# darioShar/DLPM

Measured on AMD Instinct MI355X. Metric: samples/sec at T=1000 (CIFAR-10 32x32, alpha=1.7), higher is better.
Workload: dtype f32 (1x1 / stride-2 convolutions: fp32 operands split exactly into 3 bf16 planes, bf16 MFMA products, fp32 accumulate)

## Files before the change

### dlpm_amd/csrc/conv_wino4.hip

```cpp
#include <cstdlib>
#include <type_traits>

#include "conv.h"
#include "gn_stats.h"

namespace dlpm {
namespace {

typedef float floatx4 __attribute__((ext_vector_type(4)));

constexpr int F4_TILES = 16;
constexpr int F4_NQ = 128;
constexpr int F4_KC = 8;
constexpr int F4_RAWPIX = 576;
constexpr int F4_PRLD = F4_KC + 4;
constexpr int F4_NT = 512;
constexpr int F4_QNIT = (F4_RAWPIX * 2 + F4_NT - 1) / F4_NT;
constexpr int F4_RAWBUF = F4_RAWPIX * F4_PRLD + 16;
constexpr int F4_RAWPIX_N = 400;
constexpr int F4_RAWBUF_N = F4_RAWPIX_N * F4_PRLD + 16;
constexpr int f4_nq_of(int cout) { return cout % 128 == 0 ? 128 : cout % 64 == 0 ? 64 : 32; }
constexpr int F4_CFS = 16 * 2 * F4_KC;
constexpr int F4_VBUF = 36 * F4_TILES * F4_KC;
#ifndef F4_RING_DEPTH
// ... 106 lines not shown
#pragma unroll
        for (int c = 0; c < 6; c++) Tb[c] = f4_bt_outer<5>(d, c);
        f4_v_row_out(Tb, vb + 5 * 3 * vpp, vpp);
    }
}

__device__ __forceinline__ void f4_at(float m0, float m1, float m2, float m3, float m4, float m5, float &y0, float &y1, float &y2, float &y3) {
    const float s12 = m1 + m2, d12 = m1 - m2, s34 = m3 + m4, d34 = m3 - m4;
    y0 = m0 + s12 + s34;
    y1 = fmaf(PB, d34, PA * d12);
    y2 = fmaf(PB2, s34, PA2 * s12);
    y3 = fmaf(PB3, d34, PA3 * d12) + m5;
}
__device__ __forceinline__ void f4_out_tile(const floatx4 (&acc)[36], int r, float (&Yt)[16]) {
    float Z[4][6];
#pragma unroll
    for (int b = 0; b < 6; b++)
        f4_at(acc[0 * 6 + b][r], acc[1 * 6 + b][r], acc[2 * 6 + b][r], acc[3 * 6 + b][r], acc[4 * 6 + b][r], acc[5 * 6 + b][r], Z[0][b], Z[1][b],
              Z[2][b], Z[3][b]);
#pragma unroll
    for (int i = 0; i < 4; i++) f4_at(Z[i][0], Z[i][1], Z[i][2], Z[i][3], Z[i][4], Z[i][5], Yt[i * 4 + 0], Yt[i * 4 + 1], Yt[i * 4 + 2], Yt[i * 4 + 3]);
}

template <int N>
__device__ __forceinline__ void f4_stats_lane(float K, float s1, float s2, float &mean, float &M2) {
    mean = K + s1 * (1.f / N);
    M2 = fmaxf(s2 - s1 * s1 * (1.f / N), 0.f);
}
template <int N>
__device__ __forceinline__ void f4_stats_merge(float K, float s1, float s2, int lane, float &mean, float &M2) {
    f4_stats_lane<N>(K, s1, s2, mean, M2);
    float na = (float)N;
#pragma unroll
    for (int sft = 16; sft <= 32; sft <<= 1) {
        const float om = __shfl_xor(mean, sft), oM2 = __shfl_xor(M2, sft);
        const float lo_m = (lane & sft) ? om : mean, hi_m = (lane & sft) ? mean : om;
        const float lo_M = (lane & sft) ? oM2 : M2, hi_M = (lane & sft) ? M2 : oM2;
        const float dd = hi_m - lo_m;
        mean = lo_m + dd * 0.5f;
        M2 = lo_M + hi_M + dd * dd * (na * 0.5f);
        na *= 2.f;
    }
}

__device__ __forceinline__ void f4_mfma4(float4 aa, float4 b, floatx4 &acc0, floatx4 &acc1) {
    acc0 = __builtin_amdgcn_mfma_f32_16x16x4f32(aa.x, b.x, acc0, 0, 0, 0);
    acc1 = __builtin_amdgcn_mfma_f32_16x16x4f32(aa.z, b.z, acc1, 0, 0, 0);
    acc0 = __builtin_amdgcn_mfma_f32_16x16x4f32(aa.y, b.y, acc0, 0, 0, 0);
    acc1 = __builtin_amdgcn_mfma_f32_16x16x4f32(aa.w, b.w, acc1, 0, 0, 0);
}
__device__ __forceinline__ void f4_mfma_pair(int pp, const float *asrc, int vpp, const float4 *wp, int lane, float4 (&aq)[2], float4 (&bq)[F4_RING],
                                             floatx4 (&acc)[36]) {
    constexpr int AHEAD = F4_RING - 1;
    if (pp == 0) aq[0] = *reinterpret_cast<const float4 *>(asrc);
    if (pp + AHEAD < 18) bq[(pp + AHEAD) % F4_RING] = wp[(pp + AHEAD) * 64 + lane];
    if (pp + 1 < 18) aq[(pp + 1) & 1] = *reinterpret_cast<const float4 *>(asrc + (pp + 1) * vpp);
    f4_mfma4(aq[pp & 1], bq[pp % F4_RING], acc[2 * pp], acc[2 * pp + 1]);
}

__device__ __forceinline__ float4 f4_affine4(float4 x, float4 ca, float4 cb) {
    return make_float4(fmaf(x.x, ca.x, cb.x), fmaf(x.y, ca.y, cb.y), fmaf(x.z, ca.z, cb.z), fmaf(x.w, ca.w, cb.w));
}
__device__ __forceinline__ float4 f4_silu4(float4 x) { return make_float4(silu_f(x.x), silu_f(x.y), silu_f(x.z), silu_f(x.w)); }
__device__ __forceinline__ float4 f4_affine_silu4(float4 x, float4 ca, float4 cb) { return f4_silu4(f4_affine4(x, ca, cb)); }
template <int W, int PRLD>
__device__ __forceinline__ int f4_item_pack(int pix, int ch) {
    constexpr int RW = W + 2;
    const int ry = pix / RW, rx = pix - ry * RW;
    const int iy = ry - 1, ix = rx - 1;
    const bool pad = iy < 0 || iy >= W || ix < 0 || ix >= W;
    const int lo = pix * PRLD + ch + 4 * (ry >> 2);
    return pix >= RW * RW ? (1 << 25) : (lo | (pad ? (1 << 24) : ((iy * W + ix) << 14)));
}
__device__ __forceinline__ int f4_item_lds(int iv) { return iv & 16383; }
__device__ __forceinline__ int f4_item_src(int iv) { return (iv >> 14) & 1023; }
__device__ __forceinline__ bool f4_item_pad(int iv) { return iv & (1 << 24); }
__device__ __forceinline__ bool f4_item_none(int iv) { return iv & (1 << 25); }

__device__ __forceinline__ void fs_v_row_out(const float2 (&T)[5], int ra, float *vb, int vpp) {
    const float2 e1 = f4_bt_part<1>(T[2], T[4]), o1 = f4_bt_part<1>(T[1], T[3]);
    const float2 e2 = f4_bt_part<3>(T[2], T[4]), o2 = f4_bt_part<3>(T[1], T[3]);
// ... 3 lines not shown
        const int pos = 5 * ra + rb;
        *reinterpret_cast<float2 *>(vb + (pos >> 1) * vpp + (pos & 1) * 2) = v[rb];
    }
}
template <class D>
__device__ __forceinline__ void fs_transform_rp(int rp, const D &d, float *vb, int vpp) {
    float2 Ta[5], Tb[5];
    if (rp == 0) {
#pragma unroll
        for (int c = 0; c < 5; c++) Ta[c] = f4_bt_outer<0>(d, c);
        fs_v_row_out(Ta, 0, vb, vpp);
    } else if (rp == 1) {
#pragma unroll
        for (int c = 0; c < 5; c++) f4_bt_mid<1>(d, c, Ta[c], Tb[c]);
        fs_v_row_out(Ta, 1, vb, vpp);
        fs_v_row_out(Tb, 2, vb, vpp);
    } else {
#pragma unroll
        for (int c = 0; c < 5; c++) f4_bt_mid<3>(d, c, Ta[c], Tb[c]);
        fs_v_row_out(Ta, 3, vb, vpp);
        fs_v_row_out(Tb, 4, vb, vpp);
    }
}
__device__ __forceinline__ void fs_out_tile(const floatx4 (&acc)[25], int r, float (&Yt)[16]) {
    float Z[4][5];
#pragma unroll
    for (int b = 0; b < 5; b++)
        f4_at(acc[0 * 5 + b][r], acc[1 * 5 + b][r], acc[2 * 5 + b][r], acc[3 * 5 + b][r], acc[4 * 5 + b][r], 0.f, Z[0][b], Z[1][b], Z[2][b], Z[3][b]);
#pragma unroll
    for (int i = 0; i < 4; i++) f4_at(Z[i][0], Z[i][1], Z[i][2], Z[i][3], Z[i][4], 0.f, Yt[i * 4 + 0], Yt[i * 4 + 1], Yt[i * 4 + 2], Yt[i * 4 + 3]);
}

template <bool UPS, int QN = F4_QNIT, int NW = 8>
__global__ void __launch_bounds__((NW + (NW == 8 ? 0 : NW == 4 ? 3 : 2)) * 64, NW == 2 ? 2 : 1) k_conv3x3_wino4(ConvLaunch p_in, int bh_in, int bw_in, int nimg_in) {
    constexpr bool HELP = NW != 8;
    constexpr int NH = NW == 8 ? 0 : NW == 4 ? 3 : 2;
    constexpr int F4_NT = (NW + NH) * 64, F4_NQ = NW * 16;
    constexpr int F4_RAWBUF = NW == 8 ? dlpm::F4_RAWBUF : F4_RAWBUF_N;
    ConvLaunch p = p_in;
    const int bh = bh_in, bw = bw_in, nimg = nimg_in;
    extern __shared__ __attribute__((aligned(16))) float wsm[];
    float *V = wsm;
    float *raw = wsm + 2 * F4_VBUF;
    float *Cf = raw + 2 * F4_RAWBUF;

    DLPM_PHASE_DECL;
#ifdef DLPM_PHASE_TIMING
    const long long _c0 = clock64(), _r0 = wall_clock64();
#endif
#ifdef DLPM_PHASE_TIMING
    long long _wait = 0;
#endif
    const int tid = threadIdx.x, lane = tid & 63, wave = tid >> 6;
    const bool mfma_wave = !HELP || wave < NW;
    const int li = lane & 15, lk = lane >> 4;
    const int W = p.Wout, H = p.Hout, TW = W >> 2, TH = H >> 2;
    const int Ws = UPS ? (W >> 1) : W, Hs = UPS ? (H >> 1) : H;
    const int Cin = p.C0 + p.C1;
    int nch = Cin / F4_KC, kb = 0;
    unsigned bid = blockIdx.x, nblk = gridDim.x;
    if constexpr (HELP) {
        if (p.ksplit > 1) {
            nblk = gridDim.x / p.ksplit;
            const int ks = (int)(blockIdx.x / nblk);
            bid = blockIdx.x - (unsigned)ks * nblk;
            nch /= p.ksplit;
            kb = ks * nch;
            p.out += (int64_t)ks * p.B * H * W * p.Cout;
        }
    }
    const int ntn = p.Cout / F4_NQ;
    const int nmb = nblk / ntn;
    const int mb = bid % nmb, n0 = (bid / nmb) * F4_NQ;
    int img0, ty0, tx0, blk_in_img = 0;
    if (nimg == 1) {
        const int bpr = TW / bw, bpi = (TH / bh) * bpr;
        img0 = mb / bpi;
        blk_in_img = mb - img0 * bpi;
        ty0 = (blk_in_img / bpr) * bh;
        tx0 = (blk_in_img % bpr) * bw;
    } else {
        img0 = mb * nimg;
        ty0 = tx0 = 0;
    }
    const int RH = UPS ? 2 * bh + 2 : 4 * bh + 2, RW = UPS ? 2 * bw + 2 : 4 * bw + 2;
    const int oy = UPS ? 2 * ty0 - 1 : 4 * ty0 - 1, ox = UPS ? 2 * tx0 - 1 : 4 * tx0 - 1;
    const int rpi = RH * RW, npix = nimg * rpi;

    const int squad = tid & 1;
    auto pix_of = [&](int it) { return it == 1 ? (F4_NT / 2) + ((F4_NT - 1 - tid) >> 1) : it * (F4_NT / 2) + (tid >> 1); };
    const bool skewed = !UPS && nimg == 1 && bh <= 4;
    int off[QN], lo[QN];
#pragma unroll
    for (int it = 0; it < QN; it++) {
        const int pix = pix_of(it);
        const int img = min(pix / rpi, nimg - 1), r = pix - img * rpi;
        const int ry = r / RW, rx = r - ry * RW;
        const int iy = oy + ry, ix = ox + rx;
        const bool pad = iy < 0 || iy >= Hs || ix < 0 || ix >= Ws || (img0 + img) >= p.B;
        off[it] = pix >= npix ? -2 : (pad ? -1 : (((img0 + img) * Hs + iy) * Ws + ix));
        lo[it] = (pix * F4_PRLD + squad * 4 + (skewed ? 4 * (ry >> 2) : 0)) | ((img * 2 * F4_KC + squad * 4) << 16);
    }
    const bool has_coef = p.coefA != nullptr;
    const int cf_img = tid >> 2, cf_isb = (tid >> 1) & 1;
    const bool cf_mine = has_coef && tid < nimg * 4;
    const float *cf_base = has_coef ? ((cf_isb ? p.coefB : p.coefA) + (int64_t)min(img0 + cf_img, p.B - 1) * Cin + kb * F4_KC + squad * 4) : nullptr;
    float4 xr[QN], cfr = make_float4(0.f, 0.f, 0.f, 0.f);
    auto load_raw_into = [&](float4 (&dst)[QN], int chunk) {
        const int c = (kb + chunk) * F4_KC + squad * 4;
        const bool first = c < p.C0;
        const float *sb = first ? p.src0 + c : p.src1 + (c - p.C0);
        const int ld = first ? p.C0 : p.C1;
#pragma unroll
        for (int it = 0; it < QN; it++) dst[it] = *reinterpret_cast<const float4 *>(sb + (int64_t)max(off[it], 0) * ld);
    };
    auto load_coef = [&](int chunk) {
        if (cf_mine) cfr = *reinterpret_cast<const float4 *>(cf_base + chunk * F4_KC);
    };
    auto store_coef = [&](int slot) {
        if (cf_mine) *reinterpret_cast<float4 *>(Cf + slot * F4_CFS + cf_img * 2 * F4_KC + cf_isb * F4_KC + squad * 4) = cfr;
    };
    auto store_raw_item = [&](int slot, int it) {
        if (off[it] == -2) return;
        float *rb = raw + slot * F4_RAWBUF;
        float4 x = xr[it];
        if (has_coef) {
            const float4 ca = *reinterpret_cast<const float4 *>(Cf + slot * F4_CFS + (lo[it] >> 16));
            const float4 cb = *reinterpret_cast<const float4 *>(Cf + slot * F4_CFS + (lo[it] >> 16) + F4_KC);
            x = f4_affine4(x, ca, cb);
        }
        if (p.act_silu) x = f4_silu4(x);
        if (off[it] < 0) x = make_float4(0.f, 0.f, 0.f, 0.f);
        *reinterpret_cast<float4 *>(rb + (lo[it] & 0xffff)) = x;
    };
    auto store_raw = [&](int slot) {
#pragma unroll
        for (int it = 0; it < QN; it++) store_raw_item(slot, it);
    };

    int rbase, vofs;
    {
        const int tile = lane & 15, pair = lane >> 4;
        const int timg = tile / (bh * bw), r = tile - timg * (bh * bw);
        const int ty = r / bw, tx = r - ty * bw;
        rbase = (timg * rpi + (UPS ? 2 : 4) * ty * RW + (UPS ? 2 : 4) * tx) * F4_PRLD + pair * 2 + (skewed ? 4 * ty : 0);
        vofs = (pair * F4_TILES + tile) * 4;
    }
    auto transform_rp = [&](int slot, int rp) {
        f4_transform_rp(rp, F4Patch<UPS, F4_PRLD>{raw + slot * F4_RAWBUF + rbase, RW, skewed}, V + slot * F4_VBUF + vofs, 4 * F4_TILES * 4);
    };
    auto transform = [&](int slot) {
        if (HELP) {
            if (mfma_wave) return;
            if (NH == 3) {
                transform_rp(slot, wave - NW);
            } else if (wave == NW) {
                transform_rp(slot, 0);
                transform_rp(slot, 1);
            } else {
                transform_rp(slot, 2);
            }
        } else if (wave < 3) {
            transform_rp(slot, wave);
        }
    };

    const float4 *__restrict__ wp = reinterpret_cast<const float4 *>(p.w_wino4) +
// ... 61 lines not shown
            if (pp + F4_AAHEAD < 18)
                aq[(pp + F4_AAHEAD) % (F4_AAHEAD + 1)] = *reinterpret_cast<const float4 *>(ab + (pp + F4_AAHEAD) * (4 * F4_TILES * 4));
            if (F4_PRIO) __builtin_amdgcn_s_setprio(0);
            f4_mfma4(aq[pp % (F4_AAHEAD + 1)], bq[pp % F4_RING], acc[2 * pp], acc[2 * pp + 1]);
            if (F4_PRIO) __builtin_amdgcn_s_setprio(1);
        }
        }
        store_coef(nxt);
#ifdef DLPM_PHASE_TIMING
        const long long _w0 = clock64();
#endif
        __syncthreads();
#ifdef DLPM_PHASE_TIMING
        _wait += clock64() - _w0;
#endif
    }
    if (F4_PRIO) __builtin_amdgcn_s_setprio(0);
    DLPM_PHASE(p, 9);
    if (HELP && !mfma_wave) return;
#if defined(DLPM_PHASE_TIMING) && !defined(DLPM_PHASE_DEFER)
    if (p.phase && lane == 0) atomicAdd(p.phase + 16 + wave, (unsigned long long)_wait);
#endif

    const int64_t pix0 = ((int64_t)img0 * H + 4 * ty0) * W + 4 * tx0;
    const int ch = n0 + 16 * wave + li;
    const float bias_v = p.bias ? p.bias[ch] : 0.f;
    const bool has_res = p.res0 != nullptr;
    const bool res_first = __builtin_amdgcn_readfirstlane(n0 + 16 * wave) < p.R0;
    const float *res_u = has_res ? (res_first ? p.res0 : p.res1 - p.R0) : nullptr;
    const int res_ld = res_first ? p.R0 : p.Cout - p.R0;
    const int lbw = 31 - __builtin_clz(bw), lbhw = 31 - __builtin_clz(bh * bw);
    float *__restrict__ out_blk = p.out + pix0 * p.Cout;
    const float *__restrict__ res_blk = has_res ? res_u + pix0 * res_ld : nullptr;
    const bool img_stats = p.stats_out != nullptr && nimg == 4 && bh * bw == 4;
    const bool do_stats = (p.stats_out != nullptr && nimg == 1) || img_stats;
    float K = 0.f, s1 = 0.f, s2 = 0.f;
    float rs_all[HELP ? 4 : 1][16] = {};
#pragma unroll
    for (int r = 0; r < 4; r++) {
        const int tile = 4 * lk + r;
        const int timg = tile >> lbhw, ty = (tile & (bh * bw - 1)) >> lbw, tx = tile & (bw - 1);
        const int tpix = (timg * H + 4 * ty) * W + 4 * tx;
        const bool ok = img0 + timg < p.B;
        float rs[16];
        const uint32_t bo_o = (uint32_t)(tpix * p.Cout + ch) * 4u, bo_r = (uint32_t)(tpix * res_ld + ch) * 4u;
        if (HELP) {
            if (r == 0 && has_res) {
#pragma unroll
                for (int rr = 0; rr < 4; rr++) {
                    const int t2 = 4 * lk + rr;
                    const int tp2 = ((t2 >> lbhw) * H + 4 * ((t2 & (bh * bw - 1)) >> lbw)) * W + 4 * (t2 & (bw - 1));
                    const uint32_t b2 = (uint32_t)(tp2 * res_ld + ch) * 4u;
                    const bool ok2 = img0 + (t2 >> lbhw) < p.B;
#pragma unroll
                    for (int k = 0; k < 16; k++)
                        rs_all[rr][k] = ok2 ? *reinterpret_cast<const float *>(reinterpret_cast<const char *>(res_blk + ((k >> 2) * W + (k & 3)) * res_ld) + b2) : 0.f;
                }
            }
#pragma unroll
            for (int k = 0; k < 16; k++) rs[k] = rs_all[r][k];
        } else if (has_res && ok) {
#pragma unroll
            for (int i = 0; i < 4; i++)
#pragma unroll
                for (int j = 0; j < 4; j++)
                    rs[i * 4 + j] = *reinterpret_cast<const float *>(reinterpret_cast<const char *>(res_blk + (i * W + j) * res_ld) + bo_r);
        }
        float Yt[16];
        f4_out_tile(acc, r, Yt);
        if (!ok) continue;
#pragma unroll
        for (int i = 0; i < 4; i++) {
            const float *y = Yt + 4 * i;
#pragma unroll
            for (int j = 0; j < 4; j++) {
                float v = y[j] + bias_v;
                if (has_res) v += rs[i * 4 + j];
                if (do_stats) {
                    if (r == 0 && i == 0 && j == 0) K = v;
                    const float dd = v - K;
                    s1 += dd;
                    s2 = fmaf(dd, dd, s2);
                }
                *reinterpret_cast<float *>(reinterpret_cast<char *>(out_blk + (i * W + j) * p.Cout) + bo_o) = v;
            }
        }
    }
    if (img_stats) {
        if (img0 + lk < p.B) {
            float mean, M2;
            f4_stats_lane<64>(K, s1, s2, mean, M2);
            p.stats_out[(int64_t)(img0 + lk) * p.Cout + ch] = make_float2(mean, M2);
        }
    } else if (do_stats) {
        float mean, M2;
        f4_stats_merge<64>(K, s1, s2, lane, mean, M2);
        if (lk == 0) p.stats_out[((int64_t)img0 * ((H * W) / 256) + blk_in_img) * p.Cout + ch] = make_float2(mean, M2);
    }
    DLPM_PHASE(p, 10);
    DLPM_PHASE_FLUSH(p, 8);
#ifdef DLPM_PHASE_DEFER
    if (p.phase && lane == 0) atomicAdd(p.phase + 16 + wave, (unsigned long long)_wait);
#endif
#ifdef DLPM_PHASE_TIMING
    if (p.phase && tid == 0) {
        atomicAdd(p.phase + 11, 1ull);
        atomicAdd(p.phase + 12, (unsigned long long)(clock64() - _c0));
        atomicAdd(p.phase + 13, (unsigned long long)(wall_clock64() - _r0));
    }
#endif
}

constexpr int FS_PP = 12;
constexpr int FS_FRAGS = 13;
constexpr int FS_VPP = 4 * F4_TILES * 4;
constexpr int FS_VBUF = FS_FRAGS * FS_VPP;
constexpr int FS_RAWPIX = 352;
constexpr int FS_RAWBUF = FS_RAWPIX * F4_PRLD + 16;
constexpr int FS_PAD = 16;
constexpr int FS_S0 = 4, FS_X = 9;
static_assert(FS_PP % F4_RING == 0, "a fragment's ring slot must not depend on the phase");

__global__ void __launch_bounds__(F4_NT, 1) k_conv3x3_wino4sp(ConvLaunch p_in, int bh_in, int bw_in, int nimg_in) {
    constexpr int QN = 2;
    ConvLaunch p = p_in;
    const int bh = bh_in, bw = bw_in, nimg = nimg_in;
    extern __shared__ __attribute__((aligned(16))) float wsm[];
    float *V = wsm;
    float *raw = wsm + 2 * FS_VBUF;
    float *Cf = raw + 2 * FS_RAWBUF;

    DLPM_PHASE_DECL;
#ifdef DLPM_PHASE_TIMING
    const long long _c0 = clock64(), _r0 = wall_clock64();
#endif
    const int tid = threadIdx.x, lane = tid & 63, wave = tid >> 6;
    const int li = lane & 15, lk = lane >> 4;
    const int W = p.Wout, H = p.Hout, Ws = p.Win, Hs = p.Hin, TW = Ws >> 2, TH = Hs >> 2;
    const int Cin = p.C0 + p.C1;
    const int nch = Cin / F4_KC;
    const unsigned bid = blockIdx.x;
    const int ntn = p.Cout / F4_NQ;
    const int nmb = (gridDim.x >> 2) / ntn;
    const int cls = bid & 3, mb = (bid >> 2) % nmb, nt = (bid >> 2) / nmb;
    const int ca = cls >> 1, cb = cls & 1, n0 = nt * F4_NQ;
    int img0, ty0, tx0, blk_in_img = 0;
    const int bpr = TW / bw, bpi = (TH / bh) * bpr;
    if (nimg == 1) {
        img0 = mb / bpi;
        blk_in_img = mb - img0 * bpi;
        ty0 = (blk_in_img / bpr) * bh;
        tx0 = (blk_in_img % bpr) * bw;
    } else {
        img0 = mb * nimg;
        ty0 = tx0 = 0;
    }
    const int RH = 4 * bh + 1, RW = 4 * bw + 1;
    const int oy = 4 * ty0 - 1 + ca, ox = 4 * tx0 - 1 + cb;
    const int rpi = RH * RW, npix = nimg * rpi;

    const int squad = tid & 1;
    auto pix_of = [&](int it) { return it == 1 ? (F4_NT / 2) + ((F4_NT - 1 - tid) >> 1) : (tid >> 1); };
    const bool skewed = nimg == 1 && bh <= 4;
    int off[QN], lo[QN];
#pragma unroll
    for (int it = 0; it < QN; it++) {
        const int pix = pix_of(it);
        const int img = min(pix / rpi, nimg - 1), r = pix - img * rpi;
        const int ry = r / RW, rx = r - ry * RW;
        const int iy = oy + ry, ix = ox + rx;
        const bool pad = iy < 0 || iy >= Hs || ix < 0 || ix >= Ws || (img0 + img) >= p.B;
        off[it] = pix >= npix ? -2 : (pad ? -1 : (((img0 + img) * Hs + iy) * Ws + ix));
        lo[it] = (pix * F4_PRLD + squad * 4 + (skewed ? 4 * (ry >> 2) : 0)) | ((img * 2 * F4_KC + squad * 4) << 16);
    }
    const bool has_coef = p.coefA != nullptr;
    const int cf_img = tid >> 2, cf_isb = (tid >> 1) & 1;
    const bool cf_mine = has_coef && tid < nimg * 4;
    const float *cf_base = has_coef ? ((cf_isb ? p.coefB : p.coefA) + (int64_t)min(img0 + cf_img, p.B - 1) * Cin + squad * 4) : nullptr;
    float4 xr[QN], cfr = make_float4(0.f, 0.f, 0.f, 0.f);
    auto load_raw_into = [&](float4 (&dst)[QN], int chunk) {
        const int c = chunk * F4_KC + squad * 4;
        const bool first = c < p.C0;
        const float *sb = first ? p.src0 + c : p.src1 + (c - p.C0);
        const int ld = first ? p.C0 : p.C1;
#pragma unroll
        for (int it = 0; it < QN; it++) dst[it] = *reinterpret_cast<const float4 *>(sb + (int64_t)max(off[it], 0) * ld);
    };
    auto load_coef = [&](int chunk) {
        if (cf_mine) cfr = *reinterpret_cast<const float4 *>(cf_base + chunk * F4_KC);
    };
    auto store_coef = [&](int slot) {
        if (cf_mine) *reinterpret_cast<float4 *>(Cf + slot * F4_CFS + cf_img * 2 * F4_KC + cf_isb * F4_KC + squad * 4) = cfr;
    };
    auto store_raw_item = [&](int slot, int it) {
        if (off[it] == -2) return;
        float *rb = raw + slot * FS_RAWBUF;
        float4 x = xr[it];
        if (has_coef) {
            const float4 ca4 = *reinterpret_cast<const float4 *>(Cf + slot * F4_CFS + (lo[it] >> 16));
            const float4 cb4 = *reinterpret_cast<const float4 *>(Cf + slot * F4_CFS + (lo[it] >> 16) + F4_KC);
            x = f4_affine4(x, ca4, cb4);
        }
        if (p.act_silu) x = f4_silu4(x);
        if (off[it] < 0) x = make_float4(0.f, 0.f, 0.f, 0.f);
        *reinterpret_cast<float4 *>(rb + (lo[it] & 0xffff)) = x;
    };
    auto store_raw = [&](int slot) {
#pragma unroll
        for (int it = 0; it < QN; it++) store_raw_item(slot, it);
    };

    int rbase, vofs;
    {
        const int tile = lane & 15, pair = lane >> 4;
        const int timg = tile / (bh * bw), r = tile - timg * (bh * bw);
        const int ty = r / bw, tx = r - ty * bw;
        rbase = (timg * rpi + 4 * ty * RW + 4 * tx) * F4_PRLD + pair * 2 + (skewed ? 4 * ty : 0);
        vofs = (pair * F4_TILES + tile) * 4;
    }
    auto transform = [&](int slot) {
        if (wave < 3) fs_transform_rp(wave, F4Patch<false, F4_PRLD>{raw + slot * FS_RAWBUF + rbase, RW, skewed}, V + slot * FS_VBUF + vofs, FS_VPP);
    };

    const float4 *__restrict__ wp = reinterpret_cast<const float4 *>(p.w_wino4sp) +
                                    ((int64_t)((cls * ntn + nt) * 8 + __builtin_amdgcn_readfirstlane(wave)) * nch) * FS_FRAGS * 64;
    constexpr int AHEAD = F4_RING - 1;
    float4 bq[F4_RING];
    float2 bt;
    const float *asrc = V + lane * 4;

    floatx4 acc[25];
#pragma unroll
    for (int q = 0; q < 25; q++)
#pragma unroll
        for (int r = 0; r < 4; r++) acc[q][r] = 0.f;

    const int last = nch - 1;
    float4 xr1[QN], cfr1 = make_float4(0.f, 0.f, 0.f, 0.f), cfr2 = cfr1;
    load_raw_into(xr, 0);
// ... 45 lines not shown
            if (F4_PRIO) __builtin_amdgcn_s_setprio(0);
            f4_mfma4(aq[pp & 1], bq[pp % F4_RING], acc[2 * pp], acc[2 * pp + 1]);
            if (pp == FS_PP - 1) {
                acc[24] = __builtin_amdgcn_mfma_f32_16x16x4f32(at.x, bt.x, acc[24], 0, 0, 0);
                acc[24] = __builtin_amdgcn_mfma_f32_16x16x4f32(at.y, bt.y, acc[24], 0, 0, 0);
            }
            if (F4_PRIO) __builtin_amdgcn_s_setprio(1);
        }
        bt = btn;
        wp += FS_FRAGS * 64;
        store_coef(nxt);
        __syncthreads();
    }
    if (F4_PRIO) __builtin_amdgcn_s_setprio(0);
    DLPM_PHASE(p, 9);

    const int64_t pix0 = ((int64_t)img0 * H + 8 * ty0 + ca) * W + 8 * tx0 + cb;
    const int ch = n0 + 16 * wave + li;
    const float bias_v = p.bias ? p.bias[ch] : 0.f;
    const bool has_res = p.res0 != nullptr;
    const bool res_first = __builtin_amdgcn_readfirstlane(n0 + 16 * wave) < p.R0;
    const float *res_u = has_res ? (res_first ? p.res0 : p.res1 - p.R0) : nullptr;
    const int res_ld = res_first ? p.R0 : p.Cout - p.R0;
    const int lbw = 31 - __builtin_clz(bw), lbhw = 31 - __builtin_clz(bh * bw);
    float *__restrict__ out_blk = p.out + pix0 * p.Cout;
    const float *__restrict__ res_blk = has_res ? res_u + pix0 * res_ld : nullptr;
    const bool img_stats = p.stats_out != nullptr && nimg == 4 && bh * bw == 4;
    const bool do_stats = (p.stats_out != nullptr && nimg == 1) || img_stats;
    float K = 0.f, s1 = 0.f, s2 = 0.f;
#pragma unroll
    for (int r = 0; r < 4; r++) {
        const int tile = 4 * lk + r;
        const int timg = tile >> lbhw, ty = (tile & (bh * bw - 1)) >> lbw, tx = tile & (bw - 1);
        const int tpix = (timg * H + 8 * ty) * W + 8 * tx;
        const bool ok = img0 + timg < p.B;
        float rs[16];
        const uint32_t bo_o = (uint32_t)(tpix * p.Cout + ch) * 4u, bo_r = (uint32_t)(tpix * res_ld + ch) * 4u;
        if (has_res && ok) {
#pragma unroll
            for (int i = 0; i < 4; i++)
#pragma unroll
                for (int j = 0; j < 4; j++)
                    rs[i * 4 + j] = *reinterpret_cast<const float *>(reinterpret_cast<const char *>(res_blk + (2 * i * W + 2 * j) * res_ld) + bo_r);
        }
        float Yt[16];
        fs_out_tile(acc, r, Yt);
        if (!ok) continue;
#pragma unroll
        for (int i = 0; i < 4; i++) {
            const float *y = Yt + 4 * i;
#pragma unroll
            for (int j = 0; j < 4; j++) {
                float v = y[j] + bias_v;
                if (has_res) v += rs[i * 4 + j];
                if (do_stats) {
                    if (r == 0 && i == 0 && j == 0) K = v;
                    const float dd = v - K;
                    s1 += dd;
                    s2 = fmaf(dd, dd, s2);
                }
                *reinterpret_cast<float *>(reinterpret_cast<char *>(out_blk + (2 * i * W + 2 * j) * p.Cout) + bo_o) = v;
            }
        }
    }
    if (img_stats) {
        if (img0 + lk < p.B) {
            float mean, M2;
            f4_stats_lane<64>(K, s1, s2, mean, M2);
            p.stats_out[((int64_t)(img0 + lk) * 4 + cls) * p.Cout + ch] = make_float2(mean, M2);
        }
    } else if (do_stats) {
        float mean, M2;
        f4_stats_merge<64>(K, s1, s2, lane, mean, M2);
        if (lk == 0) p.stats_out[(((int64_t)img0 * bpi + blk_in_img) * 4 + cls) * p.Cout + ch] = make_float2(mean, M2);
    }
    DLPM_PHASE(p, 10);
    DLPM_PHASE_FLUSH(p, 8);
#ifdef DLPM_PHASE_TIMING
    if (p.phase && tid == 0) {
        atomicAdd(p.phase + 11, 1ull);
        atomicAdd(p.phase + 12, (unsigned long long)(clock64() - _c0));
        atomicAdd(p.phase + 13, (unsigned long long)(wall_clock64() - _r0));
    }
#endif
}
// ... 744 lines not shown
    return v != 0 && c.Cout == 32 && !c.ups && c.Hout == 32 && c.Wout == 32 && (c.C0 + c.C1) <= 1024;
}

static int launch_conv_wino4_nq(const ConvLaunch &c, int nq, int bh, int bw, int nimg, hipStream_t st);

int launch_conv_wino4(const ConvLaunch &c, const ConvRoute &rt, hipStream_t st) {
    int bh, bw, nimg;
    if (rt.family != CONV_WINO4 || !wino4_geometry_nq(c, rt.nq, &bh, &bw, &nimg)) {
        set_error("launch_conv_wino4: unsupported shape");
        return DLPM_ERR_UNSUPPORTED;
    }
    const int nq = rt.nq;
    if (nq != f4_nq_of(c.Cout)) {
        ConvLaunch cn = c;
        cn.w_wino4 = nq == 64 ? c.w_wino4_n64 : c.w_wino4_n32;
        cn.w_wino4_n64 = cn.w_wino4_n32 = nullptr;
        cn.dispatch_B = 0;
        return launch_conv_wino4_nq(cn, nq, rt.bh, rt.bw, rt.nimg, st);
    }
    return launch_conv_wino4_nq(c, nq, rt.bh, rt.bw, rt.nimg, st);
}

static int launch_conv_wino4_nq(const ConvLaunch &c, int nq, int bh, int bw, int nimg, hipStream_t st) {
    using KFn = void (*)(ConvLaunch, int, int, int);
    const int64_t mblocks = f4_mblocks(c.B, c.Hout / 4, c.Wout / 4, nimg);
    if (wino4_whole_image(c)) {
        const int r = ensure_dynamic_lds(reinterpret_cast<const void *>(&k_conv3x3_wino4_img), 160 * 1024);
        if (r != DLPM_OK) return r;
        const size_t lds = (size_t)(FI_VBUF + FI_RAWBUF + 2 * (c.C0 + c.C1)) * sizeof(float);
        k_conv3x3_wino4_img<<<(unsigned)c.B, FI_NT, lds, st>>>(c);
        DLPM_LAUNCH_CHECK();
        return DLPM_OK;
    }
    if (nq != F4_NQ) {
        KFn fn = nq == 64 ? (c.ups ? &k_conv3x3_wino4<true, 2, 4> : &k_conv3x3_wino4<false, 2, 4>)
                          : (c.ups ? &k_conv3x3_wino4<true, 4, 2> : &k_conv3x3_wino4<false, 4, 2>);
        const int r = ensure_dynamic_lds(reinterpret_cast<const void *>(fn), 160 * 1024);
        if (r != DLPM_OK) return r;
        const size_t lds = (size_t)(2 * F4_VBUF + 2 * F4_RAWBUF_N + 2 * F4_CFS) * sizeof(float);
        const int ks = c.ksplit > 1 ? c.ksplit : 1;
        if (ks > 1 && (c.bias || c.res0 || c.stats_out || ((c.C0 + c.C1) / F4_KC) % ks != 0)) {
            set_error("launch_conv_wino4: a split-K launch carries no bias / residual / statistics and divides its chunks evenly");
            return DLPM_ERR_ARG;
        }
        fn<<<(unsigned)(mblocks * (c.Cout / nq) * ks), (nq == 64 ? 7 : 4) * 64, lds, st>>>(c, bh, bw, nimg);
        DLPM_LAUNCH_CHECK();
        return DLPM_OK;
    }
    if (c.ksplit > 1) {
        set_error("launch_conv_wino4: split-K is a narrow-shape launch");
        return DLPM_ERR_ARG;
    }
    const int RHp = c.ups ? 2 * bh + 2 : 4 * bh + 2, RWp = c.ups ? 2 * bw + 2 : 4 * bw + 2;
    const bool small = nimg * RHp * RWp <= F4_NT;
    KFn fn = c.ups ? (small ? &k_conv3x3_wino4<true, 2> : &k_conv3x3_wino4<true>) : (small ? &k_conv3x3_wino4<false, 2> : &k_conv3x3_wino4<false>);
    const int r = ensure_dynamic_lds(reinterpret_cast<const void *>(fn), 160 * 1024);
    if (r != DLPM_OK) return r;
    const size_t lds = (size_t)(2 * F4_VBUF + 2 * F4_RAWBUF + 2 * F4_CFS) * sizeof(float);
    fn<<<(unsigned)(mblocks * (c.Cout / F4_NQ)), F4_NT, lds, st>>>(c, bh, bw, nimg);
    DLPM_LAUNCH_CHECK();
    return DLPM_OK;
}

bool res_img_ok(const ResImgLaunch &r) {
    static const int v = env_switch("DLPM_RES_IMG", 1);
    const int Cin = r.C0 + r.C1;
    const bool common = v != 0 && wino4_enabled() && r.w1 && r.w2 && r.res && Cin <= 128 && Cin >= 32 &&
                        (r.st0 ? (r.C1 == 0 || r.st1 != nullptr) : (r.coefA1 && r.coefB1));
    if (r.H == 16) {
        static const int v16 = env_switch("DLPM_RES_IMG16", 1);
        return common && v16 != 0 && Cin % F6_KC == 0 && r.C0 % F6_KC == 0;
    }
    return common && r.H == 32 && r.hbuf && Cin % F4_KC == 0 && r.C0 % F4_KC == 0;
}

int launch_resblock_img(const ResImgLaunch &r, hipStream_t st) {
    if (!res_img_ok(r)) {
        set_error("launch_resblock_img: unsupported block");
        return DLPM_ERR_UNSUPPORTED;
    }
    const int Cin = r.C0 + r.C1;
#ifdef DLPM_PHASE_TIMING
// ... 57 lines not shown

bool wino4_route(const ConvLaunch &c, ConvRoute *r) {
    const int nq = wino4_nq_for(c);
    int bh, bw, nimg;
    if (!wino4_preferred(c, nq, &bh, &bw, &nimg)) return false;
    r->family = CONV_WINO4;
    if (c.ups && c.w_wino4sp && wino4sp_enabled() && nq == F4_NQ && wino4sp_geometry(c, &bh, &bw, &nimg)) r->family = CONV_WINO4SP;
    else if (c.dispatch_B > 0) r->grid = f4_mblocks(c.dispatch_B, c.Hout / 4, c.Wout / 4, nimg) * (c.Cout / nq);
    r->bh = bh; r->bw = bw; r->nimg = nimg; r->nq = nq;
    r->stats_px = nimg == 1 ? 256 : (nimg == 4 && bh * bw == 4) ? 64 : 0;
    return true;
}

int launch_conv_wino4sp(const ConvLaunch &c, const ConvRoute &rt, hipStream_t st) {
    int bh, bw, nimg;
    if (rt.family != CONV_WINO4SP || !wino4sp_geometry(c, &bh, &bw, &nimg)) {
        set_error("launch_conv_wino4sp: unsupported shape");
        return DLPM_ERR_UNSUPPORTED;
    }
    const int64_t mblocks = f4_mblocks(c.B, c.Hin / 4, c.Win / 4, rt.nimg);
    const int r = ensure_dynamic_lds(reinterpret_cast<const void *>(&k_conv3x3_wino4sp), 160 * 1024);
    if (r != DLPM_OK) return r;
    const size_t lds = (size_t)(2 * FS_VBUF + 2 * FS_RAWBUF + 2 * F4_CFS) * sizeof(float);
    k_conv3x3_wino4sp<<<(unsigned)(mblocks * (c.Cout / F4_NQ) * 4), F4_NT, lds, st>>>(c, rt.bh, rt.bw, rt.nimg);
    DLPM_LAUNCH_CHECK();
    return DLPM_OK;
}

int64_t wino4sp_weight_floats(int Cout, int Cin) { return (int64_t)4 * Cout * Cin * 26 + FS_PAD * 256; }

int relayout_weight_wino4sp(const float *oihw_dev, float *dst_dev, int Cout, int Cin, hipStream_t st) {
    const int64_t n = (int64_t)4 * Cout * Cin * 26;
    DLPM_HIP(hipMemsetAsync(dst_dev + n, 0, (size_t)FS_PAD * 256 * sizeof(float), st));
    k_relayout_weight_wino4sp<<<(unsigned)ceil_div(n, 256), 256, 0, st>>>(oihw_dev, dst_dev, Cout, Cin);
    DLPM_LAUNCH_CHECK();
    return DLPM_OK;
}

}
```

Baseline: 26.36.

## Pack Winograd output transform in pairs and use scalar-base addressing in epilogue

Reworks the conv3x3 Winograd F(4,3) epilogue so that two output tiles are inverse-transformed together with 2-wide float vectors, which lets the compiler emit packed FMA instructions. Per-pixel store and residual offsets are precomputed as uniform scalar bases plus per-lane offsets. The intent is to cut VALU work and address-computation registers in the epilogue. It also replaces integer divisions in pixel indexing with host-computed multiply-high reciprocals, checked for exactness at launch, and with shifts and masks for power-of-two tile counts. The risk is extra register pressure from holding two tiles' intermediates at once, plus a new launch-time error when a reciprocal is not exact.

```diff
diff --git a/dlpm_amd/csrc/conv_wino4.hip b/dlpm_amd/csrc/conv_wino4.hip
--- a/dlpm_amd/csrc/conv_wino4.hip
+++ b/dlpm_amd/csrc/conv_wino4.hip
@@ -152,6 +152,70 @@
     for (int i = 0; i < 4; i++) f4_at(Z[i][0], Z[i][1], Z[i][2], Z[i][3], Z[i][4], Z[i][5], Yt[i * 4 + 0], Yt[i * 4 + 1], Yt[i * 4 + 2], Yt[i * 4 + 3]);
 }
 
+typedef float floatx2 __attribute__((ext_vector_type(2)));
+__device__ __forceinline__ floatx2 f4_fma2(float a, floatx2 x, floatx2 y) { return __builtin_elementwise_fma(floatx2{a, a}, x, y); }
+__device__ __forceinline__ void f4_at2(floatx2 m0, floatx2 m1, floatx2 m2, floatx2 m3, floatx2 m4, floatx2 m5, floatx2 &y0, floatx2 &y1, floatx2 &y2,
+                                       floatx2 &y3) {
+    const floatx2 s12 = m1 + m2, d12 = m1 - m2, s34 = m3 + m4, d34 = m3 - m4;
+    y0 = m0 + s12 + s34;
+    y1 = f4_fma2(PB, d34, PA * d12);
+    y2 = f4_fma2(PB2, s34, PA2 * s12);
+    y3 = f4_fma2(PB3, d34, PA3 * d12) + m5;
+}
+template <int NPOS>
+struct F4Out2 {
+    static constexpr int N = NPOS == 36 ? 6 : 5;
+    floatx2 Z[4][N];
+    __device__ __forceinline__ void rows(const floatx4 (&acc)[NPOS], int r) {
+        const floatx2 zero = {0.f, 0.f};
+        auto m = [&](int pos) { return floatx2{acc[pos][r], acc[pos][r + 1]}; };
+#pragma unroll
+        for (int b = 0; b < N; b++)
+            f4_at2(m(0 * N + b), m(1 * N + b), m(2 * N + b), m(3 * N + b), m(4 * N + b), N == 6 ? m((N == 6 ? 5 : 0) * N + b) : zero, Z[0][b], Z[1][b],
+                   Z[2][b], Z[3][b]);
+    }
+    __device__ __forceinline__ void cols(floatx2 (&Yt)[16]) const {
+        const floatx2 zero = {0.f, 0.f};
+#pragma unroll
+        for (int i = 0; i < 4; i++)
+            f4_at2(Z[i][0], Z[i][1], Z[i][2], Z[i][3], Z[i][4], N == 6 ? Z[i][N - 1] : zero, Yt[i * 4 + 0], Yt[i * 4 + 1], Yt[i * 4 + 2], Yt[i * 4 + 3]);
+    }
+};
+typedef __attribute__((address_space(1))) char f4_gchar;
+typedef __attribute__((address_space(1))) float f4_gfloat;
+__device__ __forceinline__ f4_gchar *f4_pix_base(const void *blk, uint32_t sofs) {
+    f4_gchar *b = (f4_gchar *)(blk) + sofs;
+    asm("" : "+s"(b));
+    return b;
+}
+__device__ __forceinline__ float f4_sload(const f4_gchar *base, uint32_t vofs) { return *(const f4_gfloat *)(base + vofs); }
+__device__ __forceinline__ void f4_sstore(float v, f4_gchar *base, uint32_t vofs) { *(f4_gfloat *)(base + vofs) = v; }
+template <bool RES, bool STATS>
+__device__ __forceinline__ void f4_finish_pair(const floatx2 (&Yt)[16], const floatx2 (&rs)[16], float bias_v, const float *out, uint32_t bo0,
+                                               uint32_t bo1, const uint32_t (&so)[16], bool ok0, bool ok1, bool first, float &K, float &s1, float &s2) {
+    floatx2 v2[16];
+#pragma unroll
+    for (int k = 0; k < 16; k++) {
+        v2[k] = Yt[k] + bias_v;
+        if (RES) v2[k] += rs[k];
+    }
+#pragma unroll
+    for (int t = 0; t < 2; t++) {
+        if (!(t ? ok1 : ok0)) continue;
+#pragma unroll
+        for (int k = 0; k < 16; k++) {
+            const float v = v2[k][t];
+            if (STATS) {
+                if (first && t == 0 && k == 0) K = v;
+                const float dd = v - K;
+                s1 += dd;
+                s2 = fmaf(dd, dd, s2);
+            }
+            f4_sstore(v, f4_pix_base(out, so[k]), t ? bo1 : bo0);
+        }
+    }
+}
+
 template <int N>
 __device__ __forceinline__ void f4_stats_lane(float K, float s1, float s2, float &mean, float &M2) {
     mean = K + s1 * (1.f / N);
@@ -187,6 +251,11 @@
     if (pp + 1 < 18) aq[(pp + 1) & 1] = *reinterpret_cast<const float4 *>(asrc + (pp + 1) * vpp);
     f4_mfma4(aq[pp & 1], bq[pp % F4_RING], acc[2 * pp], acc[2 * pp + 1]);
 }
+
+__host__ __device__ constexpr uint32_t f4_rcp(int d) { return (uint32_t)(((1ull << 32) + (uint32_t)d - 1) / (uint32_t)d); }
+__host__ __device__ constexpr bool f4_rcp_exact(uint32_t m, int d, int nmax) { return (uint64_t)nmax * ((uint64_t)m * (uint32_t)d - (1ull << 32)) < (1ull << 32); }
+constexpr int F4_PIXMAX = 2 * F4_RAWPIX;
+__device__ __forceinline__ int f4_div(int n, uint32_t m) { return (int)__umulhi((uint32_t)n, m); }
 
 __device__ __forceinline__ float4 f4_affine4(float4 x, float4 ca, float4 cb) {
     return make_float4(fmaf(x.x, ca.x, cb.x), fmaf(x.y, ca.y, cb.y), fmaf(x.z, ca.z, cb.z), fmaf(x.w, ca.w, cb.w));
@@ -236,23 +305,16 @@
         fs_v_row_out(Tb, 4, vb, vpp);
     }
 }
-__device__ __forceinline__ void fs_out_tile(const floatx4 (&acc)[25], int r, float (&Yt)[16]) {
-    float Z[4][5];
-#pragma unroll
-    for (int b = 0; b < 5; b++)
-        f4_at(acc[0 * 5 + b][r], acc[1 * 5 + b][r], acc[2 * 5 + b][r], acc[3 * 5 + b][r], acc[4 * 5 + b][r], 0.f, Z[0][b], Z[1][b], Z[2][b], Z[3][b]);
-#pragma unroll
-    for (int i = 0; i < 4; i++) f4_at(Z[i][0], Z[i][1], Z[i][2], Z[i][3], Z[i][4], 0.f, Yt[i * 4 + 0], Yt[i * 4 + 1], Yt[i * 4 + 2], Yt[i * 4 + 3]);
-}
 
 template <bool UPS, int QN = F4_QNIT, int NW = 8>
-__global__ void __launch_bounds__((NW + (NW == 8 ? 0 : NW == 4 ? 3 : 2)) * 64, NW == 2 ? 2 : 1) k_conv3x3_wino4(ConvLaunch p_in, int bh_in, int bw_in, int nimg_in) {
+__global__ void __launch_bounds__((NW + (NW == 8 ? 0 : NW == 4 ? 3 : 2)) * 64, NW == 2 ? 2 : 1) k_conv3x3_wino4(ConvLaunch p_in, int bh_in, int bw_in, int nimg_in, uint32_t m_rpi, uint32_t m_rw) {
     constexpr bool HELP = NW != 8;
     constexpr int NH = NW == 8 ? 0 : NW == 4 ? 3 : 2;
     constexpr int F4_NT = (NW + NH) * 64, F4_NQ = NW * 16;
     constexpr int F4_RAWBUF = NW == 8 ? dlpm::F4_RAWBUF : F4_RAWBUF_N;
     ConvLaunch p = p_in;
     const int bh = bh_in, bw = bw_in, nimg = nimg_in;
+    const int lbw = 31 - __builtin_clz(bw), lbhw = 31 - __builtin_clz(bh * bw);
     extern __shared__ __attribute__((aligned(16))) float wsm[];
     float *V = wsm;
     float *raw = wsm + 2 * F4_VBUF;
@@ -267,7 +329,6 @@
 #endif
     const int tid = threadIdx.x, lane = tid & 63, wave = tid >> 6;
     const bool mfma_wave = !HELP || wave < NW;
-    const int li = lane & 15, lk = lane >> 4;
     const int W = p.Wout, H = p.Hout, TW = W >> 2, TH = H >> 2;
     const int Ws = UPS ? (W >> 1) : W, Hs = UPS ? (H >> 1) : H;
     const int Cin = p.C0 + p.C1;
@@ -308,8 +369,8 @@
 #pragma unroll
     for (int it = 0; it < QN; it++) {
         const int pix = pix_of(it);
-        const int img = min(pix / rpi, nimg - 1), r = pix - img * rpi;
-        const int ry = r / RW, rx = r - ry * RW;
+        const int img = min(f4_div(pix, m_rpi), nimg - 1), r = pix - img * rpi;
+        const int ry = f4_div(r, m_rw), rx = r - ry * RW;
         const int iy = oy + ry, ix = ox + rx;
         const bool pad = iy < 0 || iy >= Hs || ix < 0 || ix >= Ws || (img0 + img) >= p.B;
         off[it] = pix >= npix ? -2 : (pad ? -1 : (((img0 + img) * Hs + iy) * Ws + ix));
@@ -355,8 +416,8 @@
     int rbase, vofs;
     {
         const int tile = lane & 15, pair = lane >> 4;
-        const int timg = tile / (bh * bw), r = tile - timg * (bh * bw);
-        const int ty = r / bw, tx = r - ty * bw;
+        const int timg = tile >> lbhw, r = tile & (bh * bw - 1);
+        const int ty = r >> lbw, tx = r & (bw - 1);
         rbase = (timg * rpi + (UPS ? 2 : 4) * ty * RW + (UPS ? 2 : 4) * tx) * F4_PRLD + pair * 2 + (skewed ? 4 * ty : 0);
         vofs = (pair * F4_TILES + tile) * 4;
     }
@@ -464,6 +525,7 @@
     if (p.phase && lane == 0) atomicAdd(p.phase + 16 + wave, (unsigned long long)_wait);
 #endif
 
+    const int lane_e = __builtin_amdgcn_mbcnt_hi(~0u, __builtin_amdgcn_mbcnt_lo(~0u, 0u)), li = lane_e & 15, lk = lane_e >> 4;
     const int64_t pix0 = ((int64_t)img0 * H + 4 * ty0) * W + 4 * tx0;
     const int ch = n0 + 16 * wave + li;
     const float bias_v = p.bias ? p.bias[ch] : 0.f;
@@ -471,61 +533,55 @@
     const bool res_first = __builtin_amdgcn_readfirstlane(n0 + 16 * wave) < p.R0;
     const float *res_u = has_res ? (res_first ? p.res0 : p.res1 - p.R0) : nullptr;
     const int res_ld = res_first ? p.R0 : p.Cout - p.R0;
-    const int lbw = 31 - __builtin_clz(bw), lbhw = 31 - __builtin_clz(bh * bw);
     float *__restrict__ out_blk = p.out + pix0 * p.Cout;
     const float *__restrict__ res_blk = has_res ? res_u + pix0 * res_ld : nullptr;
     const bool img_stats = p.stats_out != nullptr && nimg == 4 && bh * bw == 4;
     const bool do_stats = (p.stats_out != nullptr && nimg == 1) || img_stats;
     float K = 0.f, s1 = 0.f, s2 = 0.f;
-    float rs_all[HELP ? 4 : 1][16] = {};
+    uint32_t so_o[16], so_r[16];
+#pragma unroll
+    for (int k = 0; k < 16; k++) {
+        so_o[k] = (uint32_t)(((k >> 2) * W + (k & 3)) * p.Cout) * 4u;
+        so_r[k] = (uint32_t)(((k >> 2) * W + (k & 3)) * res_ld) * 4u;
+    }
+    uint32_t bo_o[4], bo_r[4];
+    bool ok[4];
 #pragma unroll
     for (int r = 0; r < 4; r++) {
         const int tile = 4 * lk + r;
         const int timg = tile >> lbhw, ty = (tile & (bh * bw - 1)) >> lbw, tx = tile & (bw - 1);
         const int tpix = (timg * H + 4 * ty) * W + 4 * tx;
-        const bool ok = img0 + timg < p.B;
-        float rs[16];
-        const uint32_t bo_o = (uint32_t)(tpix * p.Cout + ch) * 4u, bo_r = (uint32_t)(tpix * res_ld + ch) * 4u;
-        if (HELP) {
-            if (r == 0 && has_res) {
-#pragma unroll
-                for (int rr = 0; rr < 4; rr++) {
-                    const int t2 = 4 * lk + rr;
-                    const int tp2 = ((t2 >> lbhw) * H + 4 * ((t2 & (bh * bw - 1)) >> lbw)) * W + 4 * (t2 & (bw - 1));
-                    const uint32_t b2 = (uint32_t)(tp2 * res_ld + ch) * 4u;
-                    const bool ok2 = img0 + (t2 >> lbhw) < p.B;
-#pragma unroll
-                    for (int k = 0; k < 16; k++)
-                        rs_all[rr][k] = ok2 ? *reinterpret_cast<const float *>(reinterpret_cast<const char *>(res_blk + ((k >> 2) * W + (k & 3)) * res_ld) + b2) : 0.f;
+        ok[r] = img0 + timg < p.B;
+        bo_o[r] = (uint32_t)(tpix * p.Cout + ch) * 4u;
+        bo_r[r] = ok[r] ? (uint32_t)(tpix * res_ld + ch) * 4u : (uint32_t)ch * 4u;
+    }
+    floatx2 rs[HELP ? 2 : 1][16];
+#pragma unroll
+    for (int rp = 0; rp < 4; rp += 2) {
+        F4Out2<36> ot;
+        if (!HELP) ot.rows(acc, rp);
+        if (has_res && (!HELP || rp == 0)) {
+#pragma unroll
+            for (int q = 0; q < (HELP ? 2 : 1); q++)
+#pragma unroll
+                for (int k = 0; k < 16; k++) {
+                    const f4_gchar *rb = f4_pix_base(res_blk, so_r[k]);
+                    rs[q][k] = floatx2{f4_sload(rb, bo_r[rp + 2 * q]), f4_sload(rb, bo_r[rp + 2 * q + 1])};
                 }
-            }
-#pragma unroll
-            for (int k = 0; k < 16; k++) rs[k] = rs_all[r][k];
-        } else if (has_res && ok) {
-#pragma unroll
-            for (int i = 0; i < 4; i++)
-#pragma unroll
-                for (int j = 0; j < 4; j++)
-                    rs[i * 4 + j] = *reinterpret_cast<const float *>(reinterpret_cast<const char *>(res_blk + (i * W + j) * res_ld) + bo_r);
-        }
-        float Yt[16];
-        f4_out_tile(acc, r, Yt);
-        if (!ok) continue;
-#pragma unroll
-        for (int i = 0; i < 4; i++) {
-            const float *y = Yt + 4 * i;
-#pragma unroll
-            for (int j = 0; j < 4; j++) {
-                float v = y[j] + bias_v;
-                if (has_res) v += rs[i * 4 + j];
-                if (do_stats) {
-                    if (r == 0 && i == 0 && j == 0) K = v;
-                    const float dd = v - K;
-                    s1 += dd;
-                    s2 = fmaf(dd, dd, s2);
-                }
-                *reinterpret_cast<float *>(reinterpret_cast<char *>(out_blk + (i * W + j) * p.Cout) + bo_o) = v;
-            }
+        }
+        if (HELP) ot.rows(acc, rp);
+        floatx2 Yt[16];
+        ot.cols(Yt);
+        auto finish = [&](auto res_c, auto stats_c) {
+            f4_finish_pair<decltype(res_c)::value, decltype(stats_c)::value>(Yt, rs[HELP ? rp >> 1 : 0], bias_v, out_blk, bo_o[rp], bo_o[rp + 1], so_o, ok[rp],
+                                                                             ok[rp + 1], rp == 0, K, s1, s2);
+        };
+        if (has_res) {
+            if (do_stats) finish(std::true_type{}, std::true_type{});
+            else finish(std::true_type{}, std::false_type{});
+        } else {
+            if (do_stats) finish(std::false_type{}, std::true_type{});
+            else finish(std::false_type{}, std::false_type{});
         }
     }
     if (img_stats) {
@@ -563,10 +619,11 @@
 constexpr int FS_S0 = 4, FS_X = 9;
 static_assert(FS_PP % F4_RING == 0, "a fragment's ring slot must not depend on the phase");
 
-__global__ void __launch_bounds__(F4_NT, 1) k_conv3x3_wino4sp(ConvLaunch p_in, int bh_in, int bw_in, int nimg_in) {
+__global__ void __launch_bounds__(F4_NT, 1) k_conv3x3_wino4sp(ConvLaunch p_in, int bh_in, int bw_in, int nimg_in, uint32_t m_rpi, uint32_t m_rw) {
     constexpr int QN = 2;
     ConvLaunch p = p_in;
     const int bh = bh_in, bw = bw_in, nimg = nimg_in;
+    const int lbw = 31 - __builtin_clz(bw), lbhw = 31 - __builtin_clz(bh * bw);
     extern __shared__ __attribute__((aligned(16))) float wsm[];
     float *V = wsm;
     float *raw = wsm + 2 * FS_VBUF;
@@ -608,8 +665,8 @@
 #pragma unroll
     for (int it = 0; it < QN; it++) {
         const int pix = pix_of(it);
-        const int img = min(pix / rpi, nimg - 1), r = pix - img * rpi;
-        const int ry = r / RW, rx = r - ry * RW;
+        const int img = min(f4_div(pix, m_rpi), nimg - 1), r = pix - img * rpi;
+        const int ry = f4_div(r, m_rw), rx = r - ry * RW;
         const int iy = oy + ry, ix = ox + rx;
         const bool pad = iy < 0 || iy >= Hs || ix < 0 || ix >= Ws || (img0 + img) >= p.B;
         off[it] = pix >= npix ? -2 : (pad ? -1 : (((img0 + img) * Hs + iy) * Ws + ix));
@@ -655,8 +712,8 @@
     int rbase, vofs;
     {
         const int tile = lane & 15, pair = lane >> 4;
-        const int timg = tile / (bh * bw), r = tile - timg * (bh * bw);
-        const int ty = r / bw, tx = r - ty * bw;
+        const int timg = tile >> lbhw, r = tile & (bh * bw - 1);
+        const int ty = r >> lbw, tx = r & (bw - 1);
         rbase = (timg * rpi + 4 * ty * RW + 4 * tx) * F4_PRLD + pair * 2 + (skewed ? 4 * ty : 0);
         vofs = (pair * F4_TILES + tile) * 4;
     }
@@ -748,45 +805,52 @@
     const bool res_first = __builtin_amdgcn_readfirstlane(n0 + 16 * wave) < p.R0;
     const float *res_u = has_res ? (res_first ? p.res0 : p.res1 - p.R0) : nullptr;
     const int res_ld = res_first ? p.R0 : p.Cout - p.R0;
-    const int lbw = 31 - __builtin_clz(bw), lbhw = 31 - __builtin_clz(bh * bw);
     float *__restrict__ out_blk = p.out + pix0 * p.Cout;
     const float *__restrict__ res_blk = has_res ? res_u + pix0 * res_ld : nullptr;
     const bool img_stats = p.stats_out != nullptr && nimg == 4 && bh * bw == 4;
     const bool do_stats = (p.stats_out != nullptr && nimg == 1) || img_stats;
     float K = 0.f, s1 = 0.f, s2 = 0.f;
+    uint32_t so_o[16], so_r[16];
+#pragma unroll
+    for (int k = 0; k < 16; k++) {
+        so_o[k] = (uint32_t)((2 * (k >> 2) * W + 2 * (k & 3)) * p.Cout) * 4u;
+        so_r[k] = (uint32_t)((2 * (k >> 2) * W + 2 * (k & 3)) * res_ld) * 4u;
+    }
+    uint32_t bo_o[4], bo_r[4];
+    bool ok[4];
 #pragma unroll
     for (int r = 0; r < 4; r++) {
         const int tile = 4 * lk + r;
         const int timg = tile >> lbhw, ty = (tile & (bh * bw - 1)) >> lbw, tx = tile & (bw - 1);
         const int tpix = (timg * H + 8 * ty) * W + 8 * tx;
-        const bool ok = img0 + timg < p.B;
-        float rs[16];
-        const uint32_t bo_o = (uint32_t)(tpix * p.Cout + ch) * 4u, bo_r = (uint32_t)(tpix * res_ld + ch) * 4u;
-        if (has_res && ok) {
-#pragma unroll
-            for (int i = 0; i < 4; i++)
-#pragma unroll
-                for (int j = 0; j < 4; j++)
-                    rs[i * 4 + j] = *reinterpret_cast<const float *>(reinterpret_cast<const char *>(res_blk + (2 * i * W + 2 * j) * res_ld) + bo_r);
-        }
-        float Yt[16];
-        fs_out_tile(acc, r, Yt);
-        if (!ok) continue;
-#pragma unroll
-        for (int i = 0; i < 4; i++) {
-            const float *y = Yt + 4 * i;
-#pragma unroll
-            for (int j = 0; j < 4; j++) {
-                float v = y[j] + bias_v;
-                if (has_res) v += rs[i * 4 + j];
-                if (do_stats) {
-                    if (r == 0 && i == 0 && j == 0) K = v;
-                    const float dd = v - K;
-                    s1 += dd;
-                    s2 = fmaf(dd, dd, s2);
-                }
-                *reinterpret_cast<float *>(reinterpret_cast<char *>(out_blk + (2 * i * W + 2 * j) * p.Cout) + bo_o) = v;
+        ok[r] = img0 + timg < p.B;
+        bo_o[r] = (uint32_t)(tpix * p.Cout + ch) * 4u;
+        bo_r[r] = ok[r] ? (uint32_t)(tpix * res_ld + ch) * 4u : (uint32_t)ch * 4u;
+    }
+    floatx2 rs[16];
+#pragma unroll
+    for (int rp = 0; rp < 4; rp += 2) {
+        F4Out2<25> ot;
+        ot.rows(acc, rp);
+        if (has_res) {
+#pragma unroll
+            for (int k = 0; k < 16; k++) {
+                const f4_gchar *rb = f4_pix_base(res_blk, so_r[k]);
+                rs[k] = floatx2{f4_sload(rb, bo_r[rp]), f4_sload(rb, bo_r[rp + 1])};
             }
+        }
+        floatx2 Yt[16];
+        ot.cols(Yt);
+        auto finish = [&](auto res_c, auto stats_c) {
+            f4_finish_pair<decltype(res_c)::value, decltype(stats_c)::value>(Yt, rs, bias_v, out_blk, bo_o[rp], bo_o[rp + 1], so_o, ok[rp], ok[rp + 1], rp == 0, K,
+                                                                             s1, s2);
+        };
+        if (has_res) {
+            if (do_stats) finish(std::true_type{}, std::true_type{});
+            else finish(std::true_type{}, std::false_type{});
+        } else {
+            if (do_stats) finish(std::false_type{}, std::true_type{});
+            else finish(std::false_type{}, std::false_type{});
         }
     }
     if (img_stats) {
@@ -1577,8 +1641,14 @@
 }
 
 static int launch_conv_wino4_nq(const ConvLaunch &c, int nq, int bh, int bw, int nimg, hipStream_t st) {
-    using KFn = void (*)(ConvLaunch, int, int, int);
+    using KFn = void (*)(ConvLaunch, int, int, int, uint32_t, uint32_t);
     const int64_t mblocks = f4_mblocks(c.B, c.Hout / 4, c.Wout / 4, nimg);
+    const int RHp = c.ups ? 2 * bh + 2 : 4 * bh + 2, RWp = c.ups ? 2 * bw + 2 : 4 * bw + 2;
+    const uint32_t m_rpi = f4_rcp(RHp * RWp), m_rw = f4_rcp(RWp);
+    if (!f4_rcp_exact(m_rpi, RHp * RWp, F4_PIXMAX) || !f4_rcp_exact(m_rw, RWp, F4_PIXMAX)) {
+        set_error("launch_conv_wino4: the reciprocal of the halo patch size is not exact over the staged pixel indices");
+        return DLPM_ERR_ARG;
+    }
     if (wino4_whole_image(c)) {
         const int r = ensure_dynamic_lds(reinterpret_cast<const void *>(&k_conv3x3_wino4_img), 160 * 1024);
         if (r != DLPM_OK) return r;
@@ -1598,7 +1668,7 @@
             set_error("launch_conv_wino4: a split-K launch carries no bias / residual / statistics and divides its chunks evenly");
             return DLPM_ERR_ARG;
         }
-        fn<<<(unsigned)(mblocks * (c.Cout / nq) * ks), (nq == 64 ? 7 : 4) * 64, lds, st>>>(c, bh, bw, nimg);
+        fn<<<(unsigned)(mblocks * (c.Cout / nq) * ks), (nq == 64 ? 7 : 4) * 64, lds, st>>>(c, bh, bw, nimg, m_rpi, m_rw);
         DLPM_LAUNCH_CHECK();
         return DLPM_OK;
     }
@@ -1606,13 +1676,12 @@
         set_error("launch_conv_wino4: split-K is a narrow-shape launch");
         return DLPM_ERR_ARG;
     }
-    const int RHp = c.ups ? 2 * bh + 2 : 4 * bh + 2, RWp = c.ups ? 2 * bw + 2 : 4 * bw + 2;
     const bool small = nimg * RHp * RWp <= F4_NT;
     KFn fn = c.ups ? (small ? &k_conv3x3_wino4<true, 2> : &k_conv3x3_wino4<true>) : (small ? &k_conv3x3_wino4<false, 2> : &k_conv3x3_wino4<false>);
     const int r = ensure_dynamic_lds(reinterpret_cast<const void *>(fn), 160 * 1024);
     if (r != DLPM_OK) return r;
     const size_t lds = (size_t)(2 * F4_VBUF + 2 * F4_RAWBUF + 2 * F4_CFS) * sizeof(float);
-    fn<<<(unsigned)(mblocks * (c.Cout / F4_NQ)), F4_NT, lds, st>>>(c, bh, bw, nimg);
+    fn<<<(unsigned)(mblocks * (c.Cout / F4_NQ)), F4_NT, lds, st>>>(c, bh, bw, nimg, m_rpi, m_rw);
     DLPM_LAUNCH_CHECK();
     return DLPM_OK;
 }
@@ -1716,7 +1785,13 @@
     const int r = ensure_dynamic_lds(reinterpret_cast<const void *>(&k_conv3x3_wino4sp), 160 * 1024);
     if (r != DLPM_OK) return r;
     const size_t lds = (size_t)(2 * FS_VBUF + 2 * FS_RAWBUF + 2 * F4_CFS) * sizeof(float);
-    k_conv3x3_wino4sp<<<(unsigned)(mblocks * (c.Cout / F4_NQ) * 4), F4_NT, lds, st>>>(c, rt.bh, rt.bw, rt.nimg);
+    const int RHs = 4 * rt.bh + 1, RWs = 4 * rt.bw + 1;
+    const uint32_t m_rpi = f4_rcp(RHs * RWs), m_rw = f4_rcp(RWs);
+    if (!f4_rcp_exact(m_rpi, RHs * RWs, F4_PIXMAX) || !f4_rcp_exact(m_rw, RWs, F4_PIXMAX)) {
+        set_error("launch_conv_wino4sp: the reciprocal of the halo patch size is not exact over the staged pixel indices");
+        return DLPM_ERR_ARG;
+    }
+    k_conv3x3_wino4sp<<<(unsigned)(mblocks * (c.Cout / F4_NQ) * 4), F4_NT, lds, st>>>(c, rt.bh, rt.bw, rt.nimg, m_rpi, m_rw);
     DLPM_LAUNCH_CHECK();
     return DLPM_OK;
 }
```

Result: no change. 26.52, median of 6 (+0.6%).
